# chenghuige/golden-huffman

Measured on AMD Instinct MI355X. Metric: encode+decode GB/s (input bytes), higher is better.
Workload: dtype u8

## Files before the change

### golden-huffman_amd/csrc/ghf_api.hip

```cpp
#include <algorithm>
#include <cstdio>
#include <cstring>
#include <new>
#include <string>

#include "ghf_code_rules.h"
#include "ghf_ctx.h"

using namespace ghf;

namespace {

thread_local std::string g_create_err;

int ensure_ws(ghf_ctx* c, size_t nchunks) {
  bool new_off = false, new_hist = false;
  int rc = grow(c, c->chunk_off, nchunks + 1, 1024, &new_off);
  if (!rc) rc = grow(c, c->chunk_hist, nchunks * 256, 1024 * 256, &new_hist);
  if (new_off) c->plan.forget();
  if (new_hist) c->hist.forget();
  return rc;
}

}
// ... 47 lines not shown
}

extern "C" {

int ghf_version(void) { return 210; }

const char* ghf_status_string(int s) {
  switch (s) {
    case GHF_OK: return "ok";
    case GHF_E_INVAL: return "invalid argument";
    case GHF_E_HIP: return "HIP runtime error / no device";
    case GHF_E_EMPTY: return "empty input (undefined in the reference)";
    case GHF_E_CODELEN: return "code longer than 32 bits (reference limit)";
    case GHF_E_CAP: return "output capacity too small";
    case GHF_E_FORMAT: return "not a .crs2 / .crs header";
    case GHF_E_CORRUPT: return "corrupt stream";
    case GHF_E_NOMEM: return "out of memory";
    case GHF_E_SINGLE: return "one distinct byte value (.crs: undefined in the reference)";
    case GHF_E_NOCODE: return "a byte value without a code in the shared code";
    default: return "unknown status";
  }
}

int ghf_ctx_create(int device, ghf_ctx** out) {
  if (!out) return GHF_E_INVAL;
  *out = nullptr;
  int ndev = 0;
  hipError_t e = hipGetDeviceCount(&ndev);
  if (e != hipSuccess || ndev <= 0) {
    g_create_err = std::string("hipGetDeviceCount: ") + (e != hipSuccess ? hipGetErrorString(e) : "no device");
    return GHF_E_HIP;
  }
  if (device < 0 || device >= ndev) return GHF_E_INVAL;
  ghf_ctx* c = new (std::nothrow) ghf_ctx();
  if (!c) return GHF_E_NOMEM;
  c->device = device;
  const char* what = "hipSetDevice";
  e = hipSetDevice(device);
#define GHF_STEP(call)      \
  if (e == hipSuccess) {    \
    what = #call;           \
    e = (call);             \
  }
  GHF_STEP(hipStreamCreateWithFlags(&c->own_stream, hipStreamNonBlocking));
  GHF_STEP(hipMalloc(&c->d_status, sizeof(int)));
  GHF_STEP(hipHostMalloc(&c->h_status, sizeof(int), hipHostMallocDefault));
  GHF_STEP(hipMalloc(&c->d_hist, GHF_NSYM * sizeof(uint64_t)));
  GHF_STEP(hipMalloc(&c->d_hist_acc, kHistAccWords * sizeof(uint64_t)));
  GHF_STEP(hipMemset(c->d_hist_acc, 0, kHistAccWords * sizeof(uint64_t)));
  GHF_STEP(hipMalloc(&c->d_code, sizeof(ghf_code)));
  GHF_STEP(hipMalloc(&c->d_tree, sizeof(ghf_tree)));
  GHF_STEP(hipMalloc(&c->d_dt, sizeof(DecTables)));
  GHF_STEP(hipMalloc(&c->d, sizeof(Scalars)));
  GHF_STEP(hipHostMalloc(&c->h, sizeof(Scalars), hipHostMallocDefault));
  GHF_STEP(hipMalloc(&c->d_planes_hist_acc, kPlanesHistAccWords * sizeof(uint64_t)));
  GHF_STEP(hipMemset(c->d_planes_hist_acc, 0, kPlanesHistAccWords * sizeof(uint64_t)));
  GHF_STEP(hipMalloc(&c->d_planes_hists, ((size_t)GHF_PLANES_MAX * GHF_NSYM + GHF_PLANES_MAX) * sizeof(uint64_t)));
  GHF_STEP(hipMalloc(&c->d_sparse_counts, kSparseGroups * sizeof(uint64_t)));
  GHF_STEP(hipMalloc(&c->d_sparse_offs, kSparseOffWords * sizeof(uint64_t)));
// ... 176 lines not shown
  size_t b = header_bytes_for(32) + (bits + 7) / 8;
  return ((b + 15) & ~(size_t)15) + 16;
}

static int histogram(ghf_ctx* c, const uint8_t* d_in, size_t n, uint64_t* d_hist, bool add) {
  if (!c || !d_hist || (n && !d_in)) return GHF_E_INVAL;
  GHF_HIP(c, hipSetDevice(c->device));
  const uint32_t cl = chunk_symbols_for(n);
  const size_t nchunks = (size_t)chunk_count_for(n);
  int rc = ensure_ws(c, nchunks);
  if (rc) return rc;
  launch_histogram(d_in, n, cl, (uint32_t)nchunks, c->chunk_hist.p, d_hist, c->d_hist_acc, add, c->stream);
  GHF_HIP(c, hipGetLastError());
  if (add) c->hist.forget();
  else c->hist = {d_in, n, cl};
  return GHF_OK;
}
int ghf_histogram(ghf_ctx* c, const uint8_t* d_in, size_t n, uint64_t* d_hist) { return histogram(c, d_in, n, d_hist, false); }
int ghf_histogram_add(ghf_ctx* c, const uint8_t* d_in, size_t n, uint64_t* d_hist) { return histogram(c, d_in, n, d_hist, true); }

int ghf_build_code_ex(ghf_ctx* c, const uint64_t* d_hist, ghf_code* d_code, unsigned flags) {
  if (!c || !d_hist || !d_code || (flags & ~(unsigned)(GHF_CODE_LIMIT | GHF_EMPTY_OK))) return GHF_E_INVAL;
  GHF_HIP(c, hipSetDevice(c->device));
  launch_build_code(d_hist, d_code, c->d_status, flags, c->stream);
  GHF_HIP(c, hipGetLastError());
  if (c->plan.code == d_code) c->plan.forget();
  if (c->prepared.describes(d_code)) c->prepared.forget();
  return GHF_OK;
}

int ghf_build_code(ghf_ctx* c, const uint64_t* d_hist, ghf_code* d_code) { return ghf_build_code_ex(c, d_hist, d_code, 0); }

int ghf_build_codes(ghf_ctx* c, const uint64_t* d_hists, uint32_t n_codes, ghf_code* d_codes, unsigned flags) {
  if (!c || !d_hists || !d_codes || n_codes == 0 || n_codes > GHF_PLANES_MAX || (flags & ~(unsigned)(GHF_CODE_LIMIT | GHF_EMPTY_OK)))
    return GHF_E_INVAL;
  GHF_HIP(c, hipSetDevice(c->device));
  launch_build_codes(d_hists, n_codes, d_codes, c->d_status, flags, c->stream);
  GHF_HIP(c, hipGetLastError());
  for (uint32_t k = 0; k < n_codes; ++k) {
    if (c->plan.code == d_codes + k) c->plan.forget();
    if (c->prepared.describes(d_codes + k)) c->prepared.forget();
  }
  return GHF_OK;
}

int ghf_write_header(ghf_ctx* c, const ghf_code* d_code, uint8_t* d_out, size_t cap) {
  if (!c || !d_code || !d_out || (reinterpret_cast<uintptr_t>(d_out) & 3u)) return GHF_E_INVAL;
  GHF_HIP(c, hipSetDevice(c->device));
  launch_write_header(d_code, d_out, cap, c->d_status, c->stream);
  GHF_HIP(c, hipGetLastError());
  return GHF_OK;
}

int ghf_encode_plan(ghf_ctx* c, const uint8_t* d_in, size_t n, const ghf_code* d_code, uint64_t* d_total_bits) {
  if (!c || !d_code || (n && !d_in)) return GHF_E_INVAL;
  GHF_HIP(c, hipSetDevice(c->device));
  const uint32_t cl = chunk_symbols_for(n);
  const size_t nchunks = (size_t)chunk_count_for(n);
  int rc = ensure_ws(c, nchunks);
  if (rc) return rc;
// ... 733 lines not shown
```

### golden-huffman_amd/csrc/ghf_batch_planes.hip

```cpp
#include "ghf_batch_core.h"
#include "ghf_build_code.h"
#include "ghf_code_rules.h"

namespace ghf {

constexpr uint32_t kHistPlaneFlushBytes = 1u << 31;
static_assert((uint64_t)kHistPlaneFlushBytes + GHF_BATCH_MAX_ITEM / 2 < (1ull << 32), "a u32 bin never wraps between two flushes");
constexpr uint32_t hist_planes_grid(uint32_t elem_bytes) { return 256u * (elem_bytes == 8 ? 4u : 8u); }

template <int E>
__global__ __launch_bounds__(kBatchThreads) void k_histogram_batch_planes(BatchPlanesHistParams P) {
  __shared__ uint32_t bins[E][kBatchWaves][256];
  const int tid = threadIdx.x, wave = tid >> 6;
#pragma unroll
  for (int p = 0; p < E; ++p)
#pragma unroll
    for (int w = 0; w < kBatchWaves; ++w) bins[p][w][tid] = 0;
  __syncthreads();
  auto flush = [&]() {
    __syncthreads();
#pragma unroll
    for (int p = 0; p < E; ++p) {
      unsigned long long c = 0;
#pragma unroll
// ... 11 lines not shown
    const uint64_t n64 = P.in_bytes[item];
    const uint8_t* __restrict__ const in = P.in_ptrs[item];
    if (n64 == 0 || n64 > P.max_item_bytes || !in || n64 % E) continue;
    const uint32_t n = (uint32_t)n64;
    const uint32_t mis = (uint32_t)reinterpret_cast<uintptr_t>(in) & 15u;
    for (uint32_t off = (uint32_t)tid * 16u; off < n; off += kBatchRoundSymbols) {
      const uint4 v = batch_load16(in, off, n, mis);
      const uint32_t cnt = n - off < 16u ? n - off : 16u;
#pragma unroll
      for (int k = 0; k < 16; ++k)
        if ((uint32_t)k < cnt) atomicAdd(&bins[k % E][wave][batch_byte(v, k)], 1u);
    }
    counted += n / E;
    if (counted > kHistPlaneFlushBytes) {
      flush();
      counted = 0;
    }
  }
  flush();
}

template <bool LIMIT>
__global__ __launch_bounds__(64) void k_build_codes(const unsigned long long* __restrict__ hists, ghf_code* __restrict__ codes,
                                                    int* __restrict__ status, uint32_t empty_ok) {
  __shared__ HeapLds heap;
  __shared__ typename std::conditional<LIMIT, LimitLds, NoLimitLds>::type Q;
  __builtin_amdgcn_s_setprio(3);
  __shared__ CodeLds cl;
  __shared__ int s_ndata;
  build_code_body<LIMIT, true>(heap, Q, cl, s_ndata, HistCounts{hists + (size_t)blockIdx.x * GHF_NSYM}, codes + blockIdx.x, status,
                               empty_ok, threadIdx.x);
}

template <int E>
__global__ __launch_bounds__(kBatchThreads) void k_compress_batch_planes_shared(BatchPlanesCompressParams P) {
  __shared__ BatchSharedCompressLds S;
  const uint32_t slot = blockIdx.x, p = slot % E;
  const BatchSharedSlot W = {P.codes + p, P.out_ptrs, P.out_caps,        P.out_bytes,     P.item_status,
                             P.chunk_bit, P.seg_bit,  P.blocks_per_item, P.segs_per_item, slot};
  PlaneItem<E> it;
  it.in_ptrs = P.in_ptrs;
  it.in_bytes = P.in_bytes;
  it.max_item_bytes = P.max_item_bytes;
  it.slot = slot;
  batch_shared_compress_body(S, W, it);
}

struct PlanesVetLds {
  unsigned long long kraft[GHF_PLANES_MAX];
  int bad;
};
template <int E>
__device__ __forceinline__ bool planes_codes_ok(PlanesVetLds& V, const ghf_code* __restrict__ codes, int tid) {
  if (tid < E) V.kraft[tid] = 0;
// ... 299 lines not shown
                                         max_len, &total, rounds, passes, StorePlane<E>{p});
    if (status == GHF_OK && have && total != n) status = GHF_E_CORRUPT;
    n = total;
    have = true;
  }
  if (tid == 0) {
    P.item_status[item] = status;
    P.out_bytes[item] = status == GHF_OK ? (uint64_t)n * E : 0;
    if (P.stats && rounds) {
      atomicAdd(reinterpret_cast<unsigned long long*>(P.stats), (unsigned long long)rounds);
      atomicAdd(reinterpret_cast<unsigned long long*>(P.stats) + 1, (unsigned long long)passes);
    }
  }
}

void launch_histogram_batch_planes(const BatchPlanesHistParams& p, uint32_t elem_bytes, uint32_t flags, hipStream_t s) {
  if (p.count == 0) return;
  (void)hipMemsetAsync(p.hists, 0, (size_t)elem_bytes * GHF_NSYM * sizeof(uint64_t), s);
  const dim3 grid(p.count < hist_planes_grid(elem_bytes) ? p.count : hist_planes_grid(elem_bytes)), block(kBatchThreads);
  with_elem_bytes(elem_bytes, [&](auto e) { hipLaunchKernelGGL(k_histogram_batch_planes<decltype(e)::value>, grid, block, 0, s, p); });
  launch_histogram_batch_finish(p.hists, elem_bytes, flags, s);
}

void launch_build_codes(const uint64_t* d_hists, uint32_t n_codes, ghf_code* d_codes, int* d_status, uint32_t flags, hipStream_t s) {
  const unsigned long long* const h = reinterpret_cast<const unsigned long long*>(d_hists);
  if (flags & GHF_CODE_LIMIT) hipLaunchKernelGGL(k_build_codes<true>, dim3(n_codes), dim3(64), 0, s, h, d_codes, d_status, flags & GHF_EMPTY_OK);
  else hipLaunchKernelGGL(k_build_codes<false>, dim3(n_codes), dim3(64), 0, s, h, d_codes, d_status, flags & GHF_EMPTY_OK);
}

void launch_batch_planes_raw_auto(const uint64_t* d_hists, const ghf_code* d_codes, uint32_t elem_bytes, uint32_t* d_raw_planes,
                                  hipStream_t s) {
  hipLaunchKernelGGL(k_batch_planes_raw_auto, dim3(1), dim3(kBatchThreads), 0, s, reinterpret_cast<const unsigned long long*>(d_hists),
                     d_codes, elem_bytes, d_raw_planes);
}

void launch_compress_batch_planes(const BatchPlanesCompressParams& p, uint32_t count, uint32_t elem_bytes, bool forms, uint32_t raw_planes,
                                  hipStream_t s) {
  if (count == 0) return;
  const dim3 grid(count * elem_bytes), block(kBatchThreads);
  with_elem_bytes(elem_bytes, [&](auto e) {
    constexpr int E = decltype(e)::value;
    if (forms) hipLaunchKernelGGL(k_compress_batch_planes_forms<E>, grid, block, 0, s, p, raw_planes);
    else hipLaunchKernelGGL(k_compress_batch_planes_shared<E>, grid, block, 0, s, p);
  });
}

void launch_decode_batch_planes(const BatchPlanesDecodeParams& p, uint32_t count, uint32_t elem_bytes, bool forms, uint32_t raw_planes,
                                hipStream_t s) {
  if (count == 0) return;
  const dim3 grid(count), block(kBatchThreads);
// ... 25 lines not shown
```

### golden-huffman_amd/csrc/ghf_build_code.h

```cpp
#ifndef GHF_BUILD_CODE_H_
#define GHF_BUILD_CODE_H_
#include <type_traits>

#include "ghf_device.h"

namespace ghf {

struct HeapLds {
  alignas(16) unsigned long long slot[528];
  uint16_t parent[GHF_NSYM + 256 + 7];
  uint16_t cur[GHF_NSYM + 3];
};

typedef unsigned long long u64t;
struct alignas(16) U64x2 { u64t x, y; };

__device__ __forceinline__ bool heap_gt(u64t a, u64t b) { return a > (b | 511ull); }

__device__ __forceinline__ void heap_sift_up(HeapLds& h, int hole, u64t e) {
  while (hole > 0) {
    const int parent = (hole - 1) >> 1;
    const u64t pe = h.slot[parent + 1];
    if (!heap_gt(pe, e)) break;
    h.slot[hole + 1] = pe;
// ... 98 lines not shown
};
__device__ __forceinline__ PushLoad wave_heap_push_load(const HeapLds& h, int n_, int lane) {
  const int n = __builtin_amdgcn_readfirstlane(n_);
  PushLoad L;
  L.depth = 31 - __clz(n + 1);
  L.on = lane >= 1 && lane <= L.depth;
  L.aj = ((n + 1) >> lane) - 1;
  L.pe = L.on ? h.slot[L.aj + 1] : 0ull;
  return L;
}
__device__ __forceinline__ void wave_heap_push_finish(HeapLds& h, const PushLoad& L, u64t e, int lane) {
  const bool stop = L.on && !heap_gt(L.pe, e);
  const unsigned long long sm = __ballot(stop);
  const int t = sm ? (__ffsll((long long)sm) - 1) - 1 : L.depth;
  const u64t up = lane_above(L.pe);
  if (lane <= t) h.slot[L.aj + 1] = (lane < t) ? up : e;
  wave_sync();
}
__device__ __forceinline__ void wave_heap_push(HeapLds& h, int n_, u64t e, int lane) {
  const PushLoad L = wave_heap_push_load(h, n_, lane);
  wave_heap_push_finish(h, L, e, lane);
}

struct CodeLds {
  uint32_t num[40];
  uint32_t first_code[64];
  uint32_t start_pos[64];
  int32_t min_len, max_len;
};

struct LimitLds {
  unsigned long long w[2][2 * GHF_NSYM];
  uint8_t is_leaf[33][2 * GHF_NSYM];
  uint16_t order[GHF_NSYM + 3];
  uint16_t len_of[34], taken[34];
  uint32_t newlen[GHF_NSYM + 3];
  long long freq[GHF_NSYM + 3];
  int n;
};

__device__ void limit_lengths_32(LimitLds& Q, const uint32_t (&len)[5], int lane) {
  constexpr int kLimit = 32;
  const long long* freq = Q.freq;
  if (lane == 0) Q.n = 0;
  __syncthreads();
#pragma unroll 1
// ... 57 lines not shown
}

struct NoLimitLds {};

template <bool ONE_WAVE_GROUP>
__device__ __forceinline__ void code_sync() {
  if constexpr (ONE_WAVE_GROUP) __syncthreads();
  else wave_sync();
}

__device__ __forceinline__ bool counts_out_of_domain(u64t mine, bool any_big) {
  if (__ballot(any_big)) return true;
#pragma unroll
  for (int d = 32; d >= 1; d >>= 1) mine += __shfl_xor(mine, d, 64);
  return (mine >> GHF_HIST_TOTAL_BITS) != 0;
}

struct HistCounts {
  static constexpr bool kAnyCount = true;
  const unsigned long long* __restrict__ hist;
  __device__ __forceinline__ long long operator()(int s) const { return (long long)hist[s]; }
};

template <bool LIMIT, bool ONE_WAVE_GROUP, class QLds, class Counts>
__device__ __forceinline__ void build_code_body(HeapLds& heap, QLds& Q, CodeLds& cl, int& s_ndata, const Counts counts,
                                                ghf_code* __restrict__ out, int* __restrict__ status, uint32_t empty_ok,
                                                const int lane) {
  long long fr[5];
#pragma unroll
  for (int j = 0; j < 5; ++j) {
    const int s = lane + 64 * j;
    fr[j] = s < GHF_NSYM ? counts(s) : 0ll;
    if constexpr (LIMIT) {
      if (s < GHF_NSYM) Q.freq[s] = fr[j];
    }
  }
  if constexpr (Counts::kAnyCount) {
    u64t mine = 0;
    bool any_big = false;
#pragma unroll
    for (int j = 0; j < 5; ++j) {
      mine += (u64t)fr[j];
      any_big |= ((u64t)fr[j] >> GHF_HIST_TOTAL_BITS) != 0;
    }
    if (counts_out_of_domain(mine, any_big)) {
      if (lane == 0) latch_status(status, GHF_E_INVAL);
      return;
    }
  }
  for (int s = lane; s < GHF_NSYM; s += 64) heap.cur[s] = (uint16_t)s;
  for (int i = lane; i < GHF_NSYM + 256 + 7; i += 64) heap.parent[i] = 0;
  if (lane < 40) cl.num[lane] = 0;
  cl.first_code[lane] = 0;
  cl.start_pos[lane] = 0;
  code_sync<ONE_WAVE_GROUP>();

  {
    int n = 0, ndata = 0;
    for (int s = 0; s < GHF_NSYM; ++s) {
      const u64t f = (u64t)__shfl(fr[s >> 6], s & 63, 64);
      if (f) {
        wave_heap_push(heap, n, (f << 9) | (u64t)s, lane);
        ++n;
        if (s < 256) ++ndata;
      }
    }
    if (lane == 0) s_ndata = ndata;
    const int times = n - 1;
    for (int t = 0; t < times; ++t) {
      const u64t e1 = wave_heap_pop(heap, n, lane);
      const u64t e2 = wave_heap_pop(heap, n, lane);
      const int s1 = (int)(e1 & 511u), s2 = (int)(e2 & 511u);
      const int node = GHF_NSYM + t;
      const PushLoad pl = wave_heap_push_load(heap, n, lane);
      const uint16_t g1 = heap.cur[s1], g2 = heap.cur[s2];
      if (lane == 0) {
        heap.parent[g1] = (uint16_t)node;
        heap.parent[g2] = (uint16_t)node;
        heap.cur[s2] = (uint16_t)node;
      }
      const u64t f = (e1 >> 9) + (e2 >> 9);
      wave_heap_push_finish(heap, pl, (f << 9) | (u64t)s2, lane);
      ++n;
    }
  }
  code_sync<ONE_WAVE_GROUP>();
  if (s_ndata == 0 && !empty_ok) {
    if (lane == 0) latch_status(status, GHF_E_EMPTY);
    return;
  }
  uint32_t len[5], node[5];
#pragma unroll
  for (int j = 0; j < 5; ++j) {
    len[j] = 0;
    node[j] = (uint32_t)(lane + 64 * j);
    if (node[j] >= GHF_NSYM) node[j] = GHF_NSYM + 256 + 1;
  }
  for (int step = 0; step < 256; ++step) {
    bool any = false;
#pragma unroll
    for (int j = 0; j < 5; ++j) {
      const uint32_t p = heap.parent[node[j]];
      if (p) {
        node[j] = p;
        len[j] += 1;
        any = true;
      }
    }
    if (!__ballot(any)) break;
  }
  if (s_ndata == 0 && lane == 0) len[4] = 1;
  uint32_t mx = 0;
#pragma unroll
  for (int j = 0; j < 5; ++j) {
    if (lane + 64 * j >= GHF_NSYM) len[j] = 0;
    mx = len[j] > mx ? len[j] : mx;
  }
#pragma unroll
  for (int d = 32; d >= 1; d >>= 1) {
    const uint32_t o = __shfl_xor(mx, d, 64);
    mx = o > mx ? o : mx;
  }
  int max_len = (int)mx;
  if (max_len > 32) {
    if constexpr (!LIMIT) {
      if (lane == 0) latch_status(status, GHF_E_CODELEN);
      return;
    } else {
      limit_lengths_32(Q, len, lane);
      mx = 0;
#pragma unroll
      for (int j = 0; j < 5; ++j) {
// ... 64 lines not shown
```

### golden-huffman_amd/csrc/ghf_ctx.h

```cpp
#ifndef GHF_CTX_H_
#define GHF_CTX_H_
#include <algorithm>
#include <cstddef>
#include <cstdint>
#include <string>

#include "ghf_internal.h"

namespace ghf {


struct K6Moved {
  uint32_t changed[2];
  unsigned long long first_inv;
};
static_assert(sizeof(K6Moved) == 16 && offsetof(K6Moved, first_inv) == 8, "one 16-byte memset clears flag, count and first");

struct K6Readback {
  uint64_t n_symbols;
  uint64_t eof_sub;
  uint64_t unused[3];
  uint64_t landing;
  K6Moved moved;
};
// ... 46 lines not shown
  bool describes(const ghf_code* code_) const { return code == code_; }
  void forget() { code = nullptr; }
};

struct RebuiltIndex {
  const uint8_t* stream = nullptr;
  size_t bytes = 0;
  bool describes(const uint8_t* stream_, size_t bytes_) const { return stream == stream_ && bytes == bytes_; }
  void forget() { stream = nullptr; }
};

}

struct ghf_ctx {
  int device = 0;
  hipStream_t own_stream = nullptr;
  hipStream_t stream = nullptr;
  int* d_status = nullptr;
  int* h_status = nullptr;
  ghf::Scalars* d = nullptr;
  ghf::Scalars* h = nullptr;
  uint64_t* d_hist = nullptr;
  uint64_t* d_hist_acc = nullptr;
  ghf_code* d_code = nullptr;
  ghf_tree* d_tree = nullptr;
  ghf::DecTables* d_dt = nullptr;
  ghf::PreparedTables prepared;
  ghf::DevBuf<uint32_t> chunk_hist;
  ghf::HistCache hist;
  ghf::DevBuf<uint64_t> chunk_off;
  ghf::PlanCache plan;
  ghf::DevBuf<uint64_t> totals;
  ghf::DevBuf<uint8_t> sync;
  ghf::DevBuf<uint32_t> seg_bit;
  ghf::DevBuf<uint64_t> seg_abs;
  ghf::DevBuf<uint64_t> chunk_bit;
  ghf_index fidx = {};
  ghf::RebuiltIndex rebuilt;
  ghf::DevBuf<uint32_t> range_seg;
  ghf::DevBuf<uint64_t> range_chunk;
  ghf::DevBuf<ghf::DecTables> range_dt;
  ghf::DevBuf<ghf_code> batch_codes;
  ghf::DevBuf<uint8_t> planes;
  uint64_t* d_planes_hist_acc = nullptr;
  uint64_t* d_planes_hists = nullptr;
  uint64_t* d_sparse_counts = nullptr;
// ... 82 lines not shown
```

### golden-huffman_amd/csrc/ghf_internal.h

```cpp
#ifndef GHF_INTERNAL_H_
#define GHF_INTERNAL_H_
#include <hip/hip_runtime.h>
#include <stdint.h>
#include <type_traits>
#include "ghf.h"

namespace ghf {

constexpr int kWave = 64;
constexpr int kSymPerLane = 16;
constexpr int kSymPerIter = kWave * kSymPerLane;
constexpr int kSegSymbols = 64;
constexpr int kBlockSymbols = 4096;
constexpr uint32_t kChunkQuantum = 4096;
constexpr uint32_t kMinChunk = 16384;
constexpr uint32_t kMaxChunk = 1u << 20;
constexpr uint32_t kEmitSlots = 256 * 3 * 8;

constexpr int kHistThreads = 256;
constexpr int kHistRep = 32;

constexpr int kEmitThreads = 512;
constexpr int kEmitWaves = kEmitThreads / kWave;
constexpr int kStageWords = 544;
// ... 324 lines not shown
struct SyncParams {
  const uint8_t* stream;
  uint64_t stream_bytes;
  uint64_t body_bit0;
  uint64_t end_bit;
  uint32_t no_eof;
  const DecTables* dt;
  uint64_t nsub;
  uint16_t* start;
  uint16_t* used;
  uint32_t* cnt;
  uint8_t* eof;
  uint32_t first;
  uint32_t first_start;
  uint32_t* changed;
  unsigned long long* moved_first_inv;
  uint64_t* eof_sub;
  uint64_t* tile_sum;
};

constexpr size_t kHistAccWords = 32 * 256 + 16 + 16 * 16;
void launch_histogram(const uint8_t* d_in, uint64_t n, uint32_t chunk, uint32_t nchunks, uint32_t* d_chunk_hist,
                      uint64_t* d_hist, uint64_t* d_acc, bool add, hipStream_t s);
void launch_build_code(const uint64_t* d_hist, ghf_code* d_code, int* d_status, uint32_t flags, hipStream_t s);
void launch_write_header(const ghf_code* d_code, uint8_t* d_out, uint64_t cap, int* d_status, hipStream_t s);
void launch_plan(const uint8_t* d_in, uint64_t n, uint32_t chunk, uint32_t nchunks, const uint32_t* d_chunk_hist,
                 const ghf_code* d_code, uint64_t* d_chunk_off, uint64_t* d_total_bits, hipStream_t s);
void launch_scan(uint64_t* d_v, uint32_t count, uint64_t* d_total, hipStream_t s);
void launch_crs_build_code(const uint64_t* d_hist, ghf_tree* d_tree, ghf_code* d_code, uint64_t* d_start_bit, int* d_status,
                           hipStream_t s);
void launch_crs_finish(const ghf_tree* d_tree, const uint64_t* d_total_bits, uint8_t* d_out, uint64_t* d_out_bytes, int* d_status,
                       hipStream_t s);
void launch_stream_copy(const uint8_t* d_src, uint8_t* d_dst, uint64_t n, bool nt, hipStream_t s);
void launch_store_u64(uint64_t* d_dst, const uint64_t* d_src_opt, uint64_t add, hipStream_t s);
void launch_load_u16(uint64_t* d_dst, const uint16_t* d_src, hipStream_t s);
void launch_shard_start(const ghf_code* d_code, const uint64_t* d_totals, int rank, uint64_t* d_start_bit, hipStream_t s);
void launch_emit(const EmitParams& p, hipStream_t s);
void launch_build_decode_tables(const ghf_code* d_code, DecTables* d_dt, int* d_status, hipStream_t s);
void launch_build_decode_tables_slots(const ghf_code* d_codes, DecTables* d_dts, uint32_t count, uint32_t slots, int* d_status, hipStream_t s);
void launch_crs_decode_tables(const ghf_tree* d_tree, DecTables* d_dt, int* d_status, hipStream_t s);
constexpr uint64_t kDecMaxGroups = 0xFFFF0000ull;
void launch_decode(const DecParams& p, hipStream_t s);
void launch_sync_pass(const SyncParams& p, hipStream_t s);
void launch_sync_counts(const SyncParams& p, uint64_t* d_total, hipStream_t s);
size_t sync_scan_workspace(uint64_t nsub);
void launch_sync_scan(const SyncParams& p, uint8_t* ws, uint32_t stride ,
                      uint32_t entry , hipStream_t s);
void launch_sync_index(const SyncParams& p, uint64_t* d_seg_abs, uint64_t n_symbols, uint64_t* d_chunk_bit, uint32_t* d_seg_bit,
                       hipStream_t s);
void launch_seek_pack(const SeekPackParams& p, hipStream_t s);
void launch_seek_expand(const SeekExpandParams& p, hipStream_t s);
void launch_seek_expand_planes(const SeekExpandPlanesParams& a, uint32_t planes, hipStream_t s);
void launch_seek_expand_streams(const SeekExpandStreamsParams& a, uint32_t streams, hipStream_t s);
void launch_decode_head(const DecHeadParams& p, hipStream_t s);
void launch_compress_batch(const BatchCompressParams& p, uint32_t count, hipStream_t s);
void launch_decode_batch(const BatchDecodeParams& p, uint32_t count, hipStream_t s);
void launch_decode_images_batch(const BatchImagesParams& p, uint32_t count, hipStream_t s);
void launch_histogram_batch(const BatchHistParams& p, uint32_t flags, hipStream_t s);
void launch_compress_batch_shared(const BatchSharedCompressParams& p, uint32_t count, hipStream_t s);
void launch_decode_batch_shared(const BatchSharedDecodeParams& p, uint32_t count, hipStream_t s);
void launch_decode_bodies_batch_shared(const BatchSharedBodiesParams& p, uint32_t count, hipStream_t s);
void launch_histogram_batch_finish(uint64_t* d_hists, uint32_t n_hists, uint32_t flags, hipStream_t s);
void launch_histogram_batch_planes(const BatchPlanesHistParams& p, uint32_t elem_bytes, uint32_t flags, hipStream_t s);
void launch_build_codes(const uint64_t* d_hists, uint32_t n_codes, ghf_code* d_codes, int* d_status, uint32_t flags, hipStream_t s);
void launch_batch_planes_raw_auto(const uint64_t* d_hists, const ghf_code* d_codes, uint32_t elem_bytes, uint32_t* d_raw_planes,
                                  hipStream_t s);
void launch_compress_batch_planes(const BatchPlanesCompressParams& p, uint32_t count, uint32_t elem_bytes, bool forms, uint32_t raw_planes,
                                  hipStream_t s);
void launch_decode_batch_planes(const BatchPlanesDecodeParams& p, uint32_t count, uint32_t elem_bytes, bool forms, uint32_t raw_planes,
                                hipStream_t s);
void launch_decode_bodies_batch_planes(const BatchPlanesBodiesParams& p, uint32_t count, uint32_t elem_bytes, bool forms,
                                       uint32_t raw_planes, hipStream_t s);
void launch_batch_seek_pack(const BatchSeekPackParams& p, uint32_t slots, hipStream_t s);
void launch_decode_bodies_batch_seek(const BatchSeekDecodeParams& p, uint32_t count, uint32_t elem_bytes, bool forms, uint32_t raw_planes,
                                     hipStream_t s);
void launch_planes_split(const uint8_t* d_in, const uint8_t* d_base, uint64_t n_elems, uint32_t elem_bytes, uint8_t* d_planes,
                         uint64_t plane_stride, hipStream_t s);
void launch_planes_merge(const uint8_t* d_planes, uint64_t plane_stride, const uint8_t* d_base, uint64_t n_elems, uint32_t elem_bytes,
                         uint8_t* d_out, const int* d_status, hipStream_t s);
void launch_planes_merge_range(const uint8_t* d_planes, uint64_t plane_stride, const uint8_t* d_base, uint64_t first, uint64_t count,
                               uint32_t elem_bytes, uint8_t* d_out, const int* d_status, hipStream_t s);
void launch_planes_split_to(const uint8_t* d_in, const uint8_t* d_base, uint64_t n_elems, uint32_t elem_bytes, uint8_t* const* h_dst,
                            hipStream_t s);
void launch_planes_merge_from(const uint8_t* const* h_src, const uint8_t* d_base, uint64_t n_elems, uint32_t elem_bytes, uint8_t* d_out,
                              const int* d_status, hipStream_t s);
void launch_sparse_split(const uint8_t* d_in, uint64_t n, uint8_t* d_mask, uint8_t* d_vals, uint64_t vals_cap, uint64_t* d_n_vals,
                         uint64_t* d_counts, uint64_t* d_offs, int* d_status, hipStream_t s);
// ... 51 lines not shown
```

### golden-huffman_amd/csrc/ghf_kernels.hip

```cpp
#include "ghf_build_code.h"

namespace ghf {

#define GHF_HADD(x, sh) atomicAdd(&lh[((((x) >> (sh)) & 0xFFu) << 5) | rep], 1u)

__device__ __forceinline__ void hist_vec(uint32_t* lh, uint32_t rep, const uint4& v) {
  GHF_HADD(v.x, 0); GHF_HADD(v.x, 8); GHF_HADD(v.x, 16); GHF_HADD(v.x, 24);
  GHF_HADD(v.y, 0); GHF_HADD(v.y, 8); GHF_HADD(v.y, 16); GHF_HADD(v.y, 24);
  GHF_HADD(v.z, 0); GHF_HADD(v.z, 8); GHF_HADD(v.z, 16); GHF_HADD(v.z, 24);
  GHF_HADD(v.w, 0); GHF_HADD(v.w, 8); GHF_HADD(v.w, 16); GHF_HADD(v.w, 24);
}

__global__ __launch_bounds__(kHistThreads) void k_histogram(const uint8_t* __restrict__ in, uint64_t n,
                                                            uint32_t chunk32, uint32_t nchunks,
                                                            uint32_t* __restrict__ chunk_hist,
                                                            unsigned long long* __restrict__ hist,
                                                            unsigned long long* __restrict__ acc ,
                                                            uint32_t add ) {
  static_assert(kHistRep == 32, "replica index is lane % 32");
  __shared__ uint32_t lh[256 * kHistRep];
  __shared__ bool s_last;
  const uint32_t tid = threadIdx.x;
  const uint32_t rep = tid & 31u;
  uint32_t prev = 0;
// ... 122 lines not shown
    }
  }
}

void launch_histogram(const uint8_t* d_in, uint64_t n, uint32_t chunk, uint32_t nchunks, uint32_t* d_chunk_hist,
                      uint64_t* d_hist, uint64_t* d_acc, bool add, hipStream_t s) {
  static int ncu = 0;
  if (ncu == 0) {
    int dev = 0;
    hipDeviceProp_t prop;
    if (hipGetDevice(&dev) == hipSuccess && hipGetDeviceProperties(&prop, dev) == hipSuccess) ncu = prop.multiProcessorCount;
    if (ncu < 1) ncu = 256;
  }
  uint32_t grid = (uint32_t)(4 * ncu);
  if (grid > nchunks) grid = nchunks;
  if (grid == 0) grid = 1;
  hipLaunchKernelGGL(k_histogram, dim3(grid), dim3(kHistThreads), 0, s, d_in, n, chunk, nchunks, d_chunk_hist,
                     reinterpret_cast<unsigned long long*>(d_hist), reinterpret_cast<unsigned long long*>(d_acc),
                     add ? 1u : 0u);
}

template <bool LIMIT>
__global__ __launch_bounds__(64) void k_build_code(const unsigned long long* __restrict__ hist, ghf_code* __restrict__ out,
                                                   int* __restrict__ status, uint32_t empty_ok) {
  __shared__ HeapLds heap;
  __shared__ typename std::conditional<LIMIT, LimitLds, NoLimitLds>::type Q;
  __builtin_amdgcn_s_setprio(3);
  __shared__ CodeLds cl;
  __shared__ int s_ndata;
  build_code_body<LIMIT, true>(heap, Q, cl, s_ndata, HistCounts{hist}, out, status, empty_ok, threadIdx.x);
}

void launch_build_code(const uint64_t* d_hist, ghf_code* d_code, int* d_status, uint32_t flags, hipStream_t s) {
  if (flags & GHF_CODE_LIMIT)
    hipLaunchKernelGGL(k_build_code<true>, dim3(1), dim3(64), 0, s, reinterpret_cast<const unsigned long long*>(d_hist), d_code, d_status,
                       flags & GHF_EMPTY_OK);
  else
    hipLaunchKernelGGL(k_build_code<false>, dim3(1), dim3(64), 0, s, reinterpret_cast<const unsigned long long*>(d_hist), d_code, d_status,
                       flags & GHF_EMPTY_OK);
}

struct TreeLds {
  uint16_t tl[256], tr[256];
  uint16_t size[GHF_NSYM + 256 + 7];
  uint8_t is_right[GHF_NSYM + 256 + 7];
  uint32_t code_hi[256];
  uint32_t max_len, min_len;
  int n;
};

__global__ __launch_bounds__(64) void k_crs_build_code(const unsigned long long* __restrict__ hist, ghf_tree* __restrict__ out_tree,
                                                       ghf_code* __restrict__ out_code, unsigned long long* __restrict__ start_bit,
                                                       int* __restrict__ status) {
  __shared__ HeapLds heap;
  __shared__ TreeLds T;
  __shared__ ghf_tree tree;
  __builtin_amdgcn_s_setprio(3);
  const int lane = threadIdx.x;
  {
    u64t mine = 0;
    bool any_big = false;
#pragma unroll
// ... 343 lines not shown
```

Baseline: 961.7.

## Add fast two-queue Huffman tree build with counting-rank sort and heap fallback

Replaces the serial wave-heap Huffman construction with a sort-then-two-queue merge. Leaves are ranked by counting comparisons across lanes, and merges are tracked in registers using readlane and scalar compares. The resulting tree is checked against the heap's tie-breaking rule using recorded tie flags and node depths, and the code falls back to the heap build if the check fails or if a hash-based tie estimate is too high. This targets the latency of the single-block code-build kernel, at the cost of extra work for the tie check and a possible second build.

```diff
diff --git a/golden-huffman_amd/csrc/ghf_api.hip b/golden-huffman_amd/csrc/ghf_api.hip
--- a/golden-huffman_amd/csrc/ghf_api.hip
+++ b/golden-huffman_amd/csrc/ghf_api.hip
@@ -93,6 +93,13 @@
   }
 }
 
+static uint32_t code_build_from_env() {
+  const char* e = getenv("GHF_CODE_BUILD");
+  if (e && !strcmp(e, "heap")) return kCodeBuildHeap;
+  if (e && !strcmp(e, "fast")) return kCodeBuildFast;
+  return kCodeBuildAuto;
+}
+
 int ghf_ctx_create(int device, ghf_ctx** out) {
   if (!out) return GHF_E_INVAL;
   *out = nullptr;
@@ -106,6 +113,7 @@
   ghf_ctx* c = new (std::nothrow) ghf_ctx();
   if (!c) return GHF_E_NOMEM;
   c->device = device;
+  c->code_build = code_build_from_env();
   const char* what = "hipSetDevice";
   e = hipSetDevice(device);
 #define GHF_STEP(call)      \
@@ -328,7 +336,7 @@
 int ghf_build_code_ex(ghf_ctx* c, const uint64_t* d_hist, ghf_code* d_code, unsigned flags) {
   if (!c || !d_hist || !d_code || (flags & ~(unsigned)(GHF_CODE_LIMIT | GHF_EMPTY_OK))) return GHF_E_INVAL;
   GHF_HIP(c, hipSetDevice(c->device));
-  launch_build_code(d_hist, d_code, c->d_status, flags, c->stream);
+  launch_build_code(d_hist, d_code, c->d_status, flags, c->code_build, c->stream);
   GHF_HIP(c, hipGetLastError());
   if (c->plan.code == d_code) c->plan.forget();
   if (c->prepared.describes(d_code)) c->prepared.forget();
@@ -341,7 +349,7 @@
   if (!c || !d_hists || !d_codes || n_codes == 0 || n_codes > GHF_PLANES_MAX || (flags & ~(unsigned)(GHF_CODE_LIMIT | GHF_EMPTY_OK)))
     return GHF_E_INVAL;
   GHF_HIP(c, hipSetDevice(c->device));
-  launch_build_codes(d_hists, n_codes, d_codes, c->d_status, flags, c->stream);
+  launch_build_codes(d_hists, n_codes, d_codes, c->d_status, flags, c->code_build, c->stream);
   GHF_HIP(c, hipGetLastError());
   for (uint32_t k = 0; k < n_codes; ++k) {
     if (c->plan.code == d_codes + k) c->plan.forget();
diff --git a/golden-huffman_amd/csrc/ghf_batch_planes.hip b/golden-huffman_amd/csrc/ghf_batch_planes.hip
--- a/golden-huffman_amd/csrc/ghf_batch_planes.hip
+++ b/golden-huffman_amd/csrc/ghf_batch_planes.hip
@@ -57,14 +57,14 @@
 
 template <bool LIMIT>
 __global__ __launch_bounds__(64) void k_build_codes(const unsigned long long* __restrict__ hists, ghf_code* __restrict__ codes,
-                                                    int* __restrict__ status, uint32_t empty_ok) {
+                                                    int* __restrict__ status, uint32_t opts) {
   __shared__ HeapLds heap;
   __shared__ typename std::conditional<LIMIT, LimitLds, NoLimitLds>::type Q;
   __builtin_amdgcn_s_setprio(3);
   __shared__ CodeLds cl;
   __shared__ int s_ndata;
-  build_code_body<LIMIT, true>(heap, Q, cl, s_ndata, HistCounts{hists + (size_t)blockIdx.x * GHF_NSYM}, codes + blockIdx.x, status,
-                               empty_ok, threadIdx.x);
+  build_code_body<LIMIT, true, true>(heap, Q, cl, s_ndata, HistCounts{hists + (size_t)blockIdx.x * GHF_NSYM}, codes + blockIdx.x,
+                                     status, code_opts_empty_ok(opts), threadIdx.x, code_opts_build(opts));
 }
 
 template <int E>
@@ -410,10 +410,11 @@
   launch_histogram_batch_finish(p.hists, elem_bytes, flags, s);
 }
 
-void launch_build_codes(const uint64_t* d_hists, uint32_t n_codes, ghf_code* d_codes, int* d_status, uint32_t flags, hipStream_t s) {
+void launch_build_codes(const uint64_t* d_hists, uint32_t n_codes, ghf_code* d_codes, int* d_status, uint32_t flags, uint32_t code_build,
+                        hipStream_t s) {
   const unsigned long long* const h = reinterpret_cast<const unsigned long long*>(d_hists);
-  if (flags & GHF_CODE_LIMIT) hipLaunchKernelGGL(k_build_codes<true>, dim3(n_codes), dim3(64), 0, s, h, d_codes, d_status, flags & GHF_EMPTY_OK);
-  else hipLaunchKernelGGL(k_build_codes<false>, dim3(n_codes), dim3(64), 0, s, h, d_codes, d_status, flags & GHF_EMPTY_OK);
+  if (flags & GHF_CODE_LIMIT) hipLaunchKernelGGL(k_build_codes<true>, dim3(n_codes), dim3(64), 0, s, h, d_codes, d_status, code_opts(flags, code_build));
+  else hipLaunchKernelGGL(k_build_codes<false>, dim3(n_codes), dim3(64), 0, s, h, d_codes, d_status, code_opts(flags, code_build));
 }
 
 void launch_batch_planes_raw_auto(const uint64_t* d_hists, const ghf_code* d_codes, uint32_t elem_bytes, uint32_t* d_raw_planes,
diff --git a/golden-huffman_amd/csrc/ghf_build_code.h b/golden-huffman_amd/csrc/ghf_build_code.h
--- a/golden-huffman_amd/csrc/ghf_build_code.h
+++ b/golden-huffman_amd/csrc/ghf_build_code.h
@@ -144,6 +144,49 @@
   wave_heap_push_finish(h, L, e, lane);
 }
 
+constexpr int kFastMaxLeafTies = 224;
+
+constexpr u64t kQueueEmpty = ~0ull;
+
+__device__ __forceinline__ u64t readlane_u64(u64t v, int l) {
+  const uint32_t lo = (uint32_t)__builtin_amdgcn_readlane((int)(uint32_t)v, l);
+  const uint32_t hi = (uint32_t)__builtin_amdgcn_readlane((int)(uint32_t)(v >> 32), l);
+  return ((u64t)hi << 32) | lo;
+}
+template <int N>
+__device__ __forceinline__ u64t spread_pick(const u64t (&a)[N], int r) {
+  u64t x = a[0];
+#pragma unroll
+  for (int k = 1; k < N; ++k)
+    if (r == k) {
+      x = a[k];
+      asm volatile("" : "+v"(x));
+    }
+  return x;
+}
+__device__ __forceinline__ bool scalar_lt_u64(u64t x, u64t y) {
+  uint32_t r;
+  asm("s_sub_u32 %0, %1, %2\n\ts_subb_u32 %0, %3, %4\n\ts_cselect_b32 %0, 1, 0"
+      : "=&s"(r)
+      : "s"(__builtin_amdgcn_readfirstlane((int)(uint32_t)x)), "s"(__builtin_amdgcn_readfirstlane((int)(uint32_t)y)),
+        "s"(__builtin_amdgcn_readfirstlane((int)(uint32_t)(x >> 32))), "s"(__builtin_amdgcn_readfirstlane((int)(uint32_t)(y >> 32)))
+      : "scc");
+  return r != 0;
+}
+
+struct MergeRec {
+  static constexpr uint32_t kIdMask = 1023u, kTieFirst = 1u << 30, kTieSecond = 1u << 31;
+  __device__ static uint32_t pack(uint32_t a, uint32_t b, uint32_t prev, bool tie_a, bool tie_b) {
+    return a | (b << 10) | (prev << 20) | (tie_a ? kTieFirst : 0u) | (tie_b ? kTieSecond : 0u);
+  }
+};
+
+struct FastTree {
+  uint32_t rec[4];
+  int times;
+  int tie_bound;
+};
+
 struct CodeLds {
   uint32_t num[40];
   uint32_t first_code[64];
@@ -247,10 +290,218 @@
   __device__ __forceinline__ long long operator()(int s) const { return (long long)hist[s]; }
 };
 
-template <bool LIMIT, bool ONE_WAVE_GROUP, class QLds, class Counts>
+__device__ __forceinline__ void heap_code_tree(HeapLds& heap, int& s_ndata, const long long (&fr)[5], const int lane) {
+  int n = 0, ndata = 0;
+  for (int s = 0; s < GHF_NSYM; ++s) {
+    const u64t f = (u64t)__shfl(fr[s >> 6], s & 63, 64);
+    if (f) {
+      wave_heap_push(heap, n, (f << 9) | (u64t)s, lane);
+      ++n;
+      if (s < 256) ++ndata;
+    }
+  }
+  if (lane == 0) s_ndata = ndata;
+  const int times = n - 1;
+  for (int t = 0; t < times; ++t) {
+    const u64t e1 = wave_heap_pop(heap, n, lane);
+    const u64t e2 = wave_heap_pop(heap, n, lane);
+    const int s1 = (int)(e1 & 511u), s2 = (int)(e2 & 511u);
+    const int node = GHF_NSYM + t;
+    const PushLoad pl = wave_heap_push_load(heap, n, lane);
+    const uint16_t g1 = heap.cur[s1], g2 = heap.cur[s2];
+    if (lane == 0) {
+      heap.parent[g1] = (uint16_t)node;
+      heap.parent[g2] = (uint16_t)node;
+      heap.cur[s2] = (uint16_t)node;
+    }
+    const u64t f = (e1 >> 9) + (e2 >> 9);
+    wave_heap_push_finish(heap, pl, (f << 9) | (u64t)s2, lane);
+    ++n;
+  }
+}
+
+template <int N>
+__device__ __forceinline__ void walk_depths(const HeapLds& heap, uint32_t (&node)[N], uint32_t (&len)[N]) {
+  for (int step = 0; step < 256; ++step) {
+    bool any = false;
+#pragma unroll
+    for (int j = 0; j < N; ++j) {
+      const uint32_t p = heap.parent[node[j]];
+      if (p) {
+        node[j] = p;
+        len[j] += 1;
+        any = true;
+      }
+    }
+    if (!__ballot(any)) break;
+  }
+}
+constexpr uint32_t kNoNode = GHF_NSYM + 256 + 1;
+
+__device__ __forceinline__ uint32_t readlane_key(uint32_t v, int l) { return (uint32_t)__builtin_amdgcn_readlane((int)v, l); }
+__device__ __forceinline__ u64t readlane_key(u64t v, int l) { return readlane_u64(v, l); }
+template <class K>
+__device__ __forceinline__ void rank_by_counting(const K (&key)[5], uint32_t (&rank)[5]) {
+#pragma unroll
+  for (int j = 0; j < 5; ++j) {
+    const int held = j < 4 ? 64 : 1;
+#pragma unroll 1
+    for (int l = 0; l < held; ++l) {
+      const K ks = readlane_key(key[j], l);
+#pragma unroll
+      for (int i = 0; i < 5; ++i) rank[i] += ks < key[i] ? 1u : 0u;
+    }
+  }
+}
+
+template <bool ONE_WAVE_GROUP>
+__device__ __forceinline__ FastTree fast_code_tree(HeapLds& heap, int& s_ndata, const long long (&fr)[5], int ties_max,
+                                                   const int lane) {
+  FastTree T;
+  T.times = 0;
+#pragma unroll
+  for (int k = 0; k < 4; ++k) T.rec[k] = 0;
+  {
+    uint32_t* bucket = reinterpret_cast<uint32_t*>(heap.slot);
+#pragma unroll
+    for (int k = 0; k < 8; ++k) heap.slot[lane + 64 * k] = 0;
+    code_sync<ONE_WAVE_GROUP>();
+    int bound = 0;
+#pragma unroll
+    for (int j = 0; j < 5; ++j) {
+      const bool live = lane + 64 * j < GHF_NSYM && fr[j] != 0;
+      const uint32_t h = ((uint32_t)fr[j] ^ (uint32_t)((u64t)fr[j] >> 32)) * 0x9E3779B1u >> 22;
+      bound += __popcll(__ballot(live && atomicAdd(&bucket[h], 1u) != 0));
+    }
+    code_sync<ONE_WAVE_GROUP>();
+    T.tie_bound = bound;
+    if (bound > ties_max) return T;
+  }
+  u64t key[5];
+  uint32_t key32[5], rank[5];
+  int nzero = 0;
+  bool big = false;
+#pragma unroll
+  for (int j = 0; j < 5; ++j) {
+    const int s = lane + 64 * j;
+    key[j] = s < GHF_NSYM ? ((u64t)fr[j] << 9) | (u64t)s : kQueueEmpty;
+    key32[j] = (uint32_t)key[j];
+    big |= s < GHF_NSYM && ((u64t)fr[j] >> 23) != 0;
+    rank[j] = 0;
+    nzero += __popcll(__ballot(s < GHF_NSYM && fr[j] == 0));
+  }
+  if (__ballot(big)) rank_by_counting(key, rank);
+  else rank_by_counting(key32, rank);
+  const int n = GHF_NSYM - nzero;
+  const int end_live = __builtin_amdgcn_readlane(fr[4] != 0 ? 1 : 0, 0);
+  if (lane == 0) s_ndata = n - end_live;
+#pragma unroll
+  for (int k = 0; k < 6; ++k) heap.slot[lane + 64 * k] = kQueueEmpty;
+  code_sync<ONE_WAVE_GROUP>();
+#pragma unroll
+  for (int j = 0; j < 5; ++j)
+    if (lane + 64 * j < GHF_NSYM && fr[j] != 0) heap.slot[rank[j] - (uint32_t)nzero] = key[j];
+  code_sync<ONE_WAVE_GROUP>();
+  u64t lw[5];
+#pragma unroll
+  for (int k = 0; k < 5; ++k) lw[k] = heap.slot[lane + 64 * k];
+
+  u64t iw[4] = {0, 0, 0, 0};
+  u64t lcur = lw[0], icur = 0;
+  int li = 0, ii = 0;
+  u64t Lk = readlane_u64(lw[0], 0), If = kQueueEmpty, prev_w = kQueueEmpty;
+  uint32_t prev_id = 0;
+  const int times = n > 1 ? n - 1 : 0;
+  int t = 0;
+  auto block = [&](auto which) __attribute__((always_inline)) {
+    constexpr int k = decltype(which)::value;
+    const int stop = times < 64 * (k + 1) ? times : 64 * (k + 1);
+#pragma unroll 1
+    for (; t < stop; ++t) {
+      u64t w[2];
+      uint32_t id[2];
+#pragma unroll
+      for (int h = 0; h < 2; ++h) {
+        const u64t Lf = Lk >> 9;
+        if (!scalar_lt_u64(If, Lf)) {
+          id[h] = (uint32_t)(Lk & 511u);
+          w[h] = Lf;
+          ++li;
+          if ((li & 63) == 0) lcur = spread_pick(lw, li >> 6);
+          Lk = readlane_u64(lcur, li & 63);
+        } else {
+          id[h] = (uint32_t)(GHF_NSYM + ii);
+          w[h] = If;
+          ++ii;
+          if ((ii & 63) == 0) icur = spread_pick(iw, ii >> 6);
+          If = ii < t ? readlane_u64(icur, ii & 63) : kQueueEmpty;
+        }
+      }
+      const u64t sum = w[0] + w[1];
+      const uint32_t r = MergeRec::pack(id[0], id[1], prev_id, w[0] == prev_w, w[1] == w[0]);
+      const bool mine = lane == (t & 63);
+      iw[k] = mine ? sum : iw[k];
+      if ((ii >> 6) == k) icur = mine ? sum : icur;
+      T.rec[k] = mine ? r : T.rec[k];
+      if (ii == t) If = sum;
+      prev_w = w[1];
+      prev_id = id[1];
+    }
+  };
+  block(std::integral_constant<int, 0>{});
+  block(std::integral_constant<int, 1>{});
+  block(std::integral_constant<int, 2>{});
+  block(std::integral_constant<int, 3>{});
+  T.times = times;
+#pragma unroll
+  for (int k = 0; k < 4; ++k) {
+    const int t = lane + 64 * k;
+    if (t < times) {
+      heap.parent[T.rec[k] & MergeRec::kIdMask] = (uint16_t)(GHF_NSYM + t);
+      heap.parent[(T.rec[k] >> 10) & MergeRec::kIdMask] = (uint16_t)(GHF_NSYM + t);
+    }
+  }
+  return T;
+}
+
+template <bool ONE_WAVE_GROUP>
+__device__ __forceinline__ bool fast_code_rule_holds(HeapLds& heap, const FastTree& T, const uint32_t (&len)[5],
+                                                     const int lane) {
+  uint16_t* depth = reinterpret_cast<uint16_t*>(heap.slot);
+  uint32_t node[4], dm[4];
+#pragma unroll
+  for (int k = 0; k < 4; ++k) {
+    const int t = lane + 64 * k;
+    node[k] = t < T.times ? (uint32_t)(GHF_NSYM + t) : kNoNode;
+    dm[k] = 0;
+  }
+  walk_depths(heap, node, dm);
+#pragma unroll
+  for (int j = 0; j < 5; ++j)
+    if (lane + 64 * j < GHF_NSYM) depth[lane + 64 * j] = (uint16_t)len[j];
+#pragma unroll
+  for (int k = 0; k < 4; ++k)
+    if (lane + 64 * k < T.times) depth[GHF_NSYM + lane + 64 * k] = (uint16_t)dm[k];
+  code_sync<ONE_WAVE_GROUP>();
+  bool bad = false;
+#pragma unroll
+  for (int k = 0; k < 4; ++k) {
+    const uint32_t r = T.rec[k];
+    if (lane + 64 * k < T.times) {
+      const uint32_t da = depth[r & MergeRec::kIdMask], db = depth[(r >> 10) & MergeRec::kIdMask];
+      const uint32_t dp = depth[(r >> 20) & MergeRec::kIdMask];
+      bad |= ((r & MergeRec::kTieFirst) && da != dp) || ((r & MergeRec::kTieSecond) && db != da);
+    }
+  }
+  const bool holds = __ballot(bad) == 0;
+  code_sync<ONE_WAVE_GROUP>();
+  return holds;
+}
+
+template <bool LIMIT, bool ONE_WAVE_GROUP, bool FAST = false, class QLds, class Counts>
 __device__ __forceinline__ void build_code_body(HeapLds& heap, QLds& Q, CodeLds& cl, int& s_ndata, const Counts counts,
                                                 ghf_code* __restrict__ out, int* __restrict__ status, uint32_t empty_ok,
-                                                const int lane) {
+                                                const int lane, const uint32_t code_build = kCodeBuildHeap) {
   long long fr[5];
 #pragma unroll
   for (int j = 0; j < 5; ++j) {
@@ -280,59 +531,44 @@
   cl.start_pos[lane] = 0;
   code_sync<ONE_WAVE_GROUP>();
 
-  {
-    int n = 0, ndata = 0;
-    for (int s = 0; s < GHF_NSYM; ++s) {
-      const u64t f = (u64t)__shfl(fr[s >> 6], s & 63, 64);
-      if (f) {
-        wave_heap_push(heap, n, (f << 9) | (u64t)s, lane);
-        ++n;
-        if (s < 256) ++ndata;
-      }
-    }
-    if (lane == 0) s_ndata = ndata;
-    const int times = n - 1;
-    for (int t = 0; t < times; ++t) {
-      const u64t e1 = wave_heap_pop(heap, n, lane);
-      const u64t e2 = wave_heap_pop(heap, n, lane);
-      const int s1 = (int)(e1 & 511u), s2 = (int)(e2 & 511u);
-      const int node = GHF_NSYM + t;
-      const PushLoad pl = wave_heap_push_load(heap, n, lane);
-      const uint16_t g1 = heap.cur[s1], g2 = heap.cur[s2];
-      if (lane == 0) {
-        heap.parent[g1] = (uint16_t)node;
-        heap.parent[g2] = (uint16_t)node;
-        heap.cur[s2] = (uint16_t)node;
-      }
-      const u64t f = (e1 >> 9) + (e2 >> 9);
-      wave_heap_push_finish(heap, pl, (f << 9) | (u64t)s2, lane);
-      ++n;
-    }
-  }
-  code_sync<ONE_WAVE_GROUP>();
+  uint32_t len[5];
+  bool fast = FAST && code_build != kCodeBuildHeap;
+  for (;;) {
+    FastTree T;
+    if constexpr (FAST) {
+      if (fast) {
+        const int ties_max = code_build == kCodeBuildFast ? GHF_NSYM : kFastMaxLeafTies;
+        T = fast_code_tree<ONE_WAVE_GROUP>(heap, s_ndata, fr, ties_max, lane);
+        fast = T.tie_bound <= ties_max;
+      }
+    }
+    if (!fast) heap_code_tree(heap, s_ndata, fr, lane);
+    code_sync<ONE_WAVE_GROUP>();
+    uint32_t node[5];
+#pragma unroll
+    for (int j = 0; j < 5; ++j) {
+      len[j] = 0;
+      node[j] = (uint32_t)(lane + 64 * j);
+      if (node[j] >= GHF_NSYM) node[j] = kNoNode;
+    }
+    walk_depths(heap, node, len);
+    if constexpr (FAST) {
+      if (fast && !fast_code_rule_holds<ONE_WAVE_GROUP>(heap, T, len, lane)) {
+        if (code_build == kCodeBuildFast) {
+          if (lane == 0) latch_status(status, GHF_E_INVAL);
+          return;
+        }
+        for (int i = lane; i < GHF_NSYM + 256 + 7; i += 64) heap.parent[i] = 0;
+        code_sync<ONE_WAVE_GROUP>();
+        fast = false;
+        continue;
+      }
+    }
+    break;
+  }
   if (s_ndata == 0 && !empty_ok) {
     if (lane == 0) latch_status(status, GHF_E_EMPTY);
     return;
-  }
-  uint32_t len[5], node[5];
-#pragma unroll
-  for (int j = 0; j < 5; ++j) {
-    len[j] = 0;
-    node[j] = (uint32_t)(lane + 64 * j);
-    if (node[j] >= GHF_NSYM) node[j] = GHF_NSYM + 256 + 1;
-  }
-  for (int step = 0; step < 256; ++step) {
-    bool any = false;
-#pragma unroll
-    for (int j = 0; j < 5; ++j) {
-      const uint32_t p = heap.parent[node[j]];
-      if (p) {
-        node[j] = p;
-        len[j] += 1;
-        any = true;
-      }
-    }
-    if (!__ballot(any)) break;
   }
   if (s_ndata == 0 && lane == 0) len[4] = 1;
   uint32_t mx = 0;
diff --git a/golden-huffman_amd/csrc/ghf_ctx.h b/golden-huffman_amd/csrc/ghf_ctx.h
--- a/golden-huffman_amd/csrc/ghf_ctx.h
+++ b/golden-huffman_amd/csrc/ghf_ctx.h
@@ -92,6 +92,7 @@
   ghf::Scalars* h = nullptr;
   uint64_t* d_hist = nullptr;
   uint64_t* d_hist_acc = nullptr;
+  uint32_t code_build = ghf::kCodeBuildAuto;
   ghf_code* d_code = nullptr;
   ghf_tree* d_tree = nullptr;
   ghf::DecTables* d_dt = nullptr;
diff --git a/golden-huffman_amd/csrc/ghf_internal.h b/golden-huffman_amd/csrc/ghf_internal.h
--- a/golden-huffman_amd/csrc/ghf_internal.h
+++ b/golden-huffman_amd/csrc/ghf_internal.h
@@ -370,7 +370,11 @@
 constexpr size_t kHistAccWords = 32 * 256 + 16 + 16 * 16;
 void launch_histogram(const uint8_t* d_in, uint64_t n, uint32_t chunk, uint32_t nchunks, uint32_t* d_chunk_hist,
                       uint64_t* d_hist, uint64_t* d_acc, bool add, hipStream_t s);
-void launch_build_code(const uint64_t* d_hist, ghf_code* d_code, int* d_status, uint32_t flags, hipStream_t s);
+enum : uint32_t { kCodeBuildAuto = 0, kCodeBuildHeap = 1, kCodeBuildFast = 2 };
+__host__ __device__ inline uint32_t code_opts(uint32_t flags, uint32_t code_build) { return (flags & GHF_EMPTY_OK) | (code_build << 8); }
+__host__ __device__ inline uint32_t code_opts_empty_ok(uint32_t opts) { return opts & GHF_EMPTY_OK; }
+__host__ __device__ inline uint32_t code_opts_build(uint32_t opts) { return opts >> 8; }
+void launch_build_code(const uint64_t* d_hist, ghf_code* d_code, int* d_status, uint32_t flags, uint32_t code_build, hipStream_t s);
 void launch_write_header(const ghf_code* d_code, uint8_t* d_out, uint64_t cap, int* d_status, hipStream_t s);
 void launch_plan(const uint8_t* d_in, uint64_t n, uint32_t chunk, uint32_t nchunks, const uint32_t* d_chunk_hist,
                  const ghf_code* d_code, uint64_t* d_chunk_off, uint64_t* d_total_bits, hipStream_t s);
@@ -410,7 +414,8 @@
 void launch_decode_bodies_batch_shared(const BatchSharedBodiesParams& p, uint32_t count, hipStream_t s);
 void launch_histogram_batch_finish(uint64_t* d_hists, uint32_t n_hists, uint32_t flags, hipStream_t s);
 void launch_histogram_batch_planes(const BatchPlanesHistParams& p, uint32_t elem_bytes, uint32_t flags, hipStream_t s);
-void launch_build_codes(const uint64_t* d_hists, uint32_t n_codes, ghf_code* d_codes, int* d_status, uint32_t flags, hipStream_t s);
+void launch_build_codes(const uint64_t* d_hists, uint32_t n_codes, ghf_code* d_codes, int* d_status, uint32_t flags, uint32_t code_build,
+                        hipStream_t s);
 void launch_batch_planes_raw_auto(const uint64_t* d_hists, const ghf_code* d_codes, uint32_t elem_bytes, uint32_t* d_raw_planes,
                                   hipStream_t s);
 void launch_compress_batch_planes(const BatchPlanesCompressParams& p, uint32_t count, uint32_t elem_bytes, bool forms, uint32_t raw_planes,
diff --git a/golden-huffman_amd/csrc/ghf_kernels.hip b/golden-huffman_amd/csrc/ghf_kernels.hip
--- a/golden-huffman_amd/csrc/ghf_kernels.hip
+++ b/golden-huffman_amd/csrc/ghf_kernels.hip
@@ -168,22 +168,22 @@
 
 template <bool LIMIT>
 __global__ __launch_bounds__(64) void k_build_code(const unsigned long long* __restrict__ hist, ghf_code* __restrict__ out,
-                                                   int* __restrict__ status, uint32_t empty_ok) {
+                                                   int* __restrict__ status, uint32_t opts) {
   __shared__ HeapLds heap;
   __shared__ typename std::conditional<LIMIT, LimitLds, NoLimitLds>::type Q;
   __builtin_amdgcn_s_setprio(3);
   __shared__ CodeLds cl;
   __shared__ int s_ndata;
-  build_code_body<LIMIT, true>(heap, Q, cl, s_ndata, HistCounts{hist}, out, status, empty_ok, threadIdx.x);
-}
-
-void launch_build_code(const uint64_t* d_hist, ghf_code* d_code, int* d_status, uint32_t flags, hipStream_t s) {
+  build_code_body<LIMIT, true, true>(heap, Q, cl, s_ndata, HistCounts{hist}, out, status, code_opts_empty_ok(opts), threadIdx.x, code_opts_build(opts));
+}
+
+void launch_build_code(const uint64_t* d_hist, ghf_code* d_code, int* d_status, uint32_t flags, uint32_t code_build, hipStream_t s) {
   if (flags & GHF_CODE_LIMIT)
     hipLaunchKernelGGL(k_build_code<true>, dim3(1), dim3(64), 0, s, reinterpret_cast<const unsigned long long*>(d_hist), d_code, d_status,
-                       flags & GHF_EMPTY_OK);
+                       code_opts(flags, code_build));
   else
     hipLaunchKernelGGL(k_build_code<false>, dim3(1), dim3(64), 0, s, reinterpret_cast<const unsigned long long*>(d_hist), d_code, d_status,
-                       flags & GHF_EMPTY_OK);
+                       code_opts(flags, code_build));
 }
 
 struct TreeLds {
```

After: 973.2, median of 6. 1.2% higher.
